# CMB-BNU/PloidyFrost

Measured on AMD Instinct MI355X. Metric: unitigs/s through superbubble+SeqAlign (k=25, z=8), higher is better.
Workload: dtype u64

## Files before the change

### ploidyfrost_amd/csrc/pf_call.hip

```cpp
#include "pf_call_kernels.hpp"
#include "pf_scan.hpp"

using namespace pf;

#define PF_TRY(call) do { const int s_ = (call); if (s_ != PF_OK) return s_; } while (0)

using namespace pf_call;

struct Need { DevBuf *buf; size_t bytes; };
static int need(pf_ctx *ctx, const char *who, std::initializer_list<Need> list) {
    for (const Need &n : list)
        if (!n.buf->ensure(n.bytes)) { pf::CtxErr{ctx} = std::string(who) + ": out of device memory"; return PF_ERR_HIP; }
    return PF_OK;
}

namespace pf {

void call_state_create(pf_ctx *ctx) { (void)state_of(ctx); }
void call_destroy(pf_ctx *ctx) {
    if (!ctx->call) return;
    ctx->call->release_all();
    delete ctx->call;
    ctx->call = nullptr;
}
// ... 242 lines not shown
    PF_HIP(hipMemcpyAsync(&total, S->side_base.as<uint32_t>() + N, 4, hipMemcpyDeviceToHost, st));
    PF_HIP(hipStreamSynchronize(st));
    S->n_sides = total;
    S->n_tasks = 0;
    S->low = lower;
    S->up = upper;
    *n_sides = total;
    if (total == 0) return PF_OK;
    if (!S->sides.ensure((size_t)total * sizeof(pf_call_side)) || !S->ctask.ensure((size_t)total * sizeof(CallTask)) ||
        !S->target.ensure((size_t)total * 4)) {
        pf::CtxErr{ctx} = "pf_call_scan: out of device memory";
        return PF_ERR_HIP;
    }
    ScanArgs a;
    a.flags = S->flags.as<uint8_t>(); a.plus = S->plus.as<uint32_t>(); a.minus = S->minus.as<uint32_t>();
    a.succ = ctx->d_succ; a.pred = ctx->d_pred; a.seq = ctx->d_seq; a.off = ctx->d_off; a.len = ctx->d_len; a.N = N; a.k = ctx->k;
    a.cov_sum = S->cov_sum.as<uint64_t>(); a.cov_min = S->cov_min.as<uint32_t>(); a.cov_miss = S->cov_miss.as<uint8_t>();
    a.per_strand = S->per_strand; a.low = lower; a.up = upper;
    a.side_base = S->side_base.as<uint32_t>(); a.sides = S->sides.as<pf_call_side>(); a.tasks = S->ctask.as<CallTask>();
    a.target = S->target.as<uint32_t>();
    a.n_colors = S->n_colors;
    a.ccov_sum = S->ccov_sum.as<uint64_t>(); a.ccov_min = S->ccov_min.as<uint32_t>(); a.ccov_max = S->ccov_max.as<uint32_t>(); a.ccov_miss = S->ccov_miss.as<uint8_t>();
    a.clow = S->col_low.as<uint32_t>(); a.cup = S->col_up.as<uint32_t>(); a.full = S->col_full.as<uint64_t>(); a.cwords = S->col_words; a.size_total = S->col_size.as<uint64_t>();
    ctx_begin(ctx, PF_K_CALL_SCAN);
    if (S->n_colors) k_call_sides<true><<<(N + 255) / 256, 256, 0, st>>>(a);
    else k_call_sides<false><<<(N + 255) / 256, 256, 0, st>>>(a);
    ctx_end(ctx);
    ctx_units(ctx, PF_K_CALL_SCAN, N);
    PF_HIP(hipGetLastError());
    return PF_OK;
}

int pf_call_resolve(pf_ctx *ctx, uint64_t *n_bubbles, uint32_t *err, uint32_t *err_unitig) {
    if (!ctx || !ctx->call || !n_bubbles || !err || !err_unitig) return PF_ERR_ARG;
    CallState *S = ctx->call;
    *n_bubbles = 0;
    *err = 0;
    *err_unitig = 0;
    S->n_tasks = 0;
    const uint64_t n = S->n_sides;
    if (n == 0) return PF_OK;
    PF_HIP(hipSetDevice(ctx->device));
    hipStream_t st = ctx->stream;
    if (!S->pending.ensure(n * 4) || !S->killed.ensure(n) || !S->rstate.ensure(n) || !S->rflag.ensure(n * 4) || !S->rsmall.ensure(64) ||
        !S->kept.ensure(n * 4)) {
        pf::CtxErr{ctx} = "pf_call_resolve: out of device memory";
// ... 878 lines not shown
```

### ploidyfrost_amd/csrc/pf_colored.hip

```cpp
#include <hip/hip_runtime.h>

#include <algorithm>
#include <cstdlib>
#include <cstring>
#include <string>
#include <vector>

#include "pf_colored_dev.hpp"
#include "pf_cov_stream.hpp"
#include "pf_ctx.hpp"
#include "pf_device_common.hpp"
#include "ploidyfrost_hip.h"

using namespace pf;

namespace {

constexpr uint32_t MISSING = pf::CTAB_MISSING;

__global__ void k_ctab_build(uint8_t *base, uint64_t mask, uint32_t line_bytes, int k, const uint64_t *__restrict__ kmers,
                             const uint32_t *__restrict__ counts, uint64_t n, uint64_t min_count, uint64_t max_count, uint32_t colour,
                             unsigned int *noncanon) {
    uint64_t i = (uint64_t)blockIdx.x * blockDim.x + threadIdx.x;
    const uint64_t stride = (uint64_t)gridDim.x * blockDim.x;
// ... 317 lines not shown
        ctx->n_colors, ctx->n_kmers, ctx->d_gcov_c, stride, rest, rest_n, rest_cap, ROWS)
        if (ctx->k == 25) PF_JOINC_LAUNCH(25);
        else if (ctx->k == 31) PF_JOINC_LAUNCH(31);
        else PF_JOINC_LAUNCH(0);
#undef PF_JOINC_LAUNCH
        ctx_end_at(ctx, at, st);
        (void)ctx_begin_at(ctx, PF_K_COV_JOIN_REST, st, &at);
        k_cov_join_colored_rest<<<blocks, 256, 0, st>>>(t, ctx->k, ctx->n_colors, rest, rest_n, rest_cap, ctx->d_gcov_c, stride, ctx->d_seq, ctx->d_off,
                                                                  ctx->d_kpre, ctx->d_khead, ctx->d_krow, ctx->n_kmers, ROWS);
        ctx_end_at(ctx, at, st);
    } else {
        (void)ctx_begin_at(ctx, PF_K_COV_JOIN, st, &at);
        k_cov_colored<<<ctx_grid(ctx, (uint64_t)ctx->N * 64, 256, 16), 256, 0, st>>>(t, ctx->d_seq, ctx->d_off, ctx->d_len, ctx->k, ctx->ctab_one_strand,
                                                                                            ctx->n_colors, 0, ctx->N, ctx->d_unread, nullptr, nullptr,
                                                                                            nullptr, nullptr, ctx->d_kpre, ctx->d_gcov_c, stride);
        ctx_end_at(ctx, at, st);
    }
    PF_HIP(hipGetLastError());
    PF_HIP(hipEventRecord(ctx->join_c_done, st));
    ctx->join_c_inflight = true;
    return PF_OK;
}

int join_colored_finish(pf_ctx *ctx) {
    if (!ctx->join_c_inflight) return PF_OK;
    ctx->join_c_inflight = false;
    PF_HIP(hipSetDevice(ctx->device));
    PF_HIP(hipEventSynchronize(ctx->join_c_done));
    ctx->gcov_c_valid = true;
    return PF_OK;
}

int join_graph_counts_colored(pf_ctx *ctx) {
    const int rc = join_graph_counts_colored_begin(ctx);
    return rc ? rc : join_colored_finish(ctx);
}
}

extern "C" {

uint32_t pf_num_colors(const pf_ctx *ctx) { return ctx ? ctx->n_colors : 0; }

int pf_upload_counts_colored(pf_ctx *ctx, uint32_t n_colors, const uint64_t *const *kmers, const uint32_t *const *counts,
                             const uint64_t *n, const uint64_t *min_count, const uint64_t *max_count, const int *both_strands) {
    if (!ctx || n_colors == 0 || !kmers || !counts || !n || !min_count || !max_count || !both_strands) return PF_ERR_ARG;
    if (n_colors > PF_MAX_COLORS_TABLE) { pf::CtxErr{ctx} = "more colours than the device table holds (PF_MAX_COLORS_TABLE)"; return PF_ERR_ARG; }
    if (!ctx->d_seq || !ctx->k) { pf::CtxErr{ctx} = "pf_upload_counts_colored: the graph comes first (the table is addressed by minimizers of length-k keys)"; return PF_ERR_ARG; }
    uint64_t total = 0, biggest = 0;
    for (uint32_t c = 0; c < n_colors; ++c) {
        if (n[c] && (!kmers[c] || !counts[c])) return PF_ERR_ARG;
        if (!both_strands[c]) continue;
        total += n[c];
        biggest = std::max(biggest, n[c]);
    }
    ctx->ctab_unread = 0;
    ctx->ctab_max_count = 0;
    std::vector<uint8_t> unread(n_colors, 0);
    for (uint32_t c = 0; c < n_colors; ++c) {
        if (!both_strands[c]) { unread[c] = 1; if (c < 64) ctx->ctab_unread |= 1ull << c; }
        else ctx->ctab_max_count = std::max<uint64_t>(ctx->ctab_max_count, max_count[c]);
    }
    (void)join_colored_finish(ctx);
    if (ctx->d_gcov_c) { (void)hipFree(ctx->d_gcov_c); ctx->d_gcov_c = nullptr; }
    ctx->gcov_c_valid = false;
    PF_HIP(hipSetDevice(ctx->device));
    if (ctx->d_ctab) { (void)hipFree(ctx->d_ctab); ctx->d_ctab = nullptr; }
    if (ctx->d_unread) { (void)hipFree(ctx->d_unread); ctx->d_unread = nullptr; }
    PF_HIP(hipMalloc(reinterpret_cast<void **>(&ctx->d_unread), n_colors));
    PF_HIP(hipMemcpy(ctx->d_unread, unread.data(), n_colors, hipMemcpyHostToDevice));
    ctx->n_colors = 0;
    uint64_t cap = 128;
    while (cap * 4 < biggest || cap * LINE_KEYS < total + total / 4 + 1) cap <<= 1;
    const uint32_t line_bytes = ctab_line_bytes(n_colors);
    PF_HIP(hipMalloc(reinterpret_cast<void **>(&ctx->d_ctab), cap * line_bytes));
    PF_HIP(hipMemsetAsync(ctx->d_ctab, 0xFF, cap * line_bytes, ctx->stream));
    ctx->ctab_cap = cap;
    ctx->ctab_line_bytes = line_bytes;
    DevTmp<unsigned int> noncanon_;
    PF_HIP(noncanon_.alloc(4));
    PF_HIP(hipMemsetAsync(noncanon_.p, 0, 4, ctx->stream));
    for (uint32_t c = 0; c < n_colors; ++c) {
        if (!n[c] || !both_strands[c]) continue;
        DevTmp<uint64_t> dk_;
        DevTmp<uint32_t> dc_;
        const uint64_t *pk = kmers[c];
// ... 28 lines not shown
    }
    ctx->n_colors = n_colors;
    return join_graph_counts_colored(ctx);
}

static int unitig_cov_colored_impl(pf_ctx *ctx, uint32_t u0, uint32_t u1, uint64_t *sum, uint32_t *mn, uint32_t *mx, uint8_t *miss, bool probe) {
    if (!ctx || !ctx->d_seq || !ctx->d_ctab || !ctx->n_colors || u0 > u1 || u1 > ctx->N || !sum || !mn || !mx || !miss) return PF_ERR_ARG;
    if (u0 == u1) return PF_OK;
    PF_HIP(hipSetDevice(ctx->device));
    const size_t n = (size_t)(u1 - u0) * ctx->n_colors;
    const bool dev_out = on_device(sum);
    uint64_t *ds = sum;
    uint32_t *dlo = mn, *dhi = mx;
    uint8_t *dx = miss;
    if (!dev_out) {
        ds = (uint64_t *)ctx_ws(ctx, WS_CCOV_SUM, n * 8);
        dlo = (uint32_t *)ctx_ws(ctx, WS_CCOV_MIN, n * 4);
        dhi = (uint32_t *)ctx_ws(ctx, WS_CCOV_MAX, n * 4);
        dx = (uint8_t *)ctx_ws(ctx, WS_CCOV_MISS, n);
        if (!ds || !dlo || !dhi || !dx) return PF_ERR_HIP;
    }
    constexpr bool env_probe = false;
    probe = probe || env_probe;
    { const int rc = join_colored_finish(ctx); if (rc) return rc; }
    if (!probe && !ctx->gcov_c_valid) {
        const int rc = join_graph_counts_colored(ctx);
        if (rc) return rc;
    }
    const bool stream = !probe && ctx->gcov_c_valid;
    uint64_t g_range[2] = {0, 0};
    if (stream) {
        PF_HIP(hipMemcpyAsync(&g_range[0], ctx->d_kpre + u0, 8, hipMemcpyDeviceToHost, ctx->stream));
        PF_HIP(hipMemcpyAsync(&g_range[1], ctx->d_kpre + u1, 8, hipMemcpyDeviceToHost, ctx->stream));
        PF_HIP(hipStreamSynchronize(ctx->stream));
    }
    ctx_begin(ctx, PF_K_COV_COLORED);
    if (stream) {
        k_ccov_init<<<ctx_grid(ctx, n, 256, 8), 256, 0, ctx->stream>>>(n, ds, dlo, dhi, dx);
        Kc4Args a{ctx->d_gcov_c, ctx->gcov_c_stride, ctx->d_unread, ctx->d_khead, ctx->d_krow, u0, u1 - u0, g_range[0], g_range[1],
                  g_range[0] / 256, (g_range[1] + 255) / 256, ds, dlo, dhi, dx};
        const int rc = launch_cov_stream(ctx, a, ctx->n_colors, ctx->ctab_max_count >= (1ull << 20), true);
        if (rc) return rc;
    } else {
        const CTab t{ctx->d_ctab, ctx->ctab_cap - 1, ctx->ctab_line_bytes};
        const int grid = ctx_grid(ctx, (uint64_t)(u1 - u0) * 64, 256, 16);
        k_cov_colored<<<grid, 256, 0, ctx->stream>>>(t, ctx->d_seq, ctx->d_off, ctx->d_len, ctx->k, ctx->ctab_one_strand, ctx->n_colors, u0, u1,
                                                     ctx->d_unread, ds, dlo, dhi, dx, nullptr, nullptr, 0);
    }
    ctx_end(ctx);
    if (!dev_out) {
        PF_HIP(hipMemcpyAsync(sum, ds, n * 8, hipMemcpyDeviceToHost, ctx->stream));
        PF_HIP(hipMemcpyAsync(mn, dlo, n * 4, hipMemcpyDeviceToHost, ctx->stream));
        PF_HIP(hipMemcpyAsync(mx, dhi, n * 4, hipMemcpyDeviceToHost, ctx->stream));
        PF_HIP(hipMemcpyAsync(miss, dx, n, hipMemcpyDeviceToHost, ctx->stream));
        PF_HIP(hipStreamSynchronize(ctx->stream));
    }
    return PF_OK;
}

int pf_unitig_cov_colored(pf_ctx *ctx, uint32_t u0, uint32_t u1, uint64_t *sum, uint32_t *mn, uint32_t *mx, uint8_t *miss) {
    return unitig_cov_colored_impl(ctx, u0, u1, sum, mn, mx, miss, false);
}

int pf_unitig_cov_colored_probe(pf_ctx *ctx, uint32_t u0, uint32_t u1, uint64_t *sum, uint32_t *mn, uint32_t *mx, uint8_t *miss) {
    return unitig_cov_colored_impl(ctx, u0, u1, sum, mn, mx, miss, true);
}

int pf_string_cov_colored(pf_ctx *ctx, const char *text, const uint64_t *str_off, uint32_t n_str, const uint32_t *low,
                          const uint32_t *up, uint64_t *sum, uint8_t *ok) {
    if (!ctx || !ctx->d_ctab || !ctx->n_colors || !low || !up || (n_str && (!text || !str_off || !sum || !ok))) return PF_ERR_ARG;
    if (n_str == 0) return PF_OK;
    PF_HIP(hipSetDevice(ctx->device));
    const uint32_t C = ctx->n_colors;
    uint64_t total = 0;
    PF_HIP(hipMemcpy(&total, str_off + n_str, 8, hipMemcpyDefault));
    char *dt = (char *)ctx_ws(ctx, WS_STR_TEXT, (size_t)total + 1);
    uint64_t *doff = (uint64_t *)ctx_ws(ctx, WS_STR_OFF, ((size_t)n_str + 1) * 8);
    uint64_t *ds = (uint64_t *)ctx_ws(ctx, WS_STR_SUM, (size_t)n_str * C * 8);
// ... 20 lines not shown
```

### ploidyfrost_amd/csrc/pf_ctx.hpp

```cpp
#pragma once
#include <hip/hip_runtime.h>
#include <stdint.h>

#include <mutex>
#include <string>
#include <vector>

#include "pf_device_common.hpp"
#include "ploidyfrost_hip.h"

namespace pf {
template <typename T>
struct DevTmp {
    T *p = nullptr;
    DevTmp() = default;
    DevTmp(const DevTmp &) = delete;
    DevTmp &operator=(const DevTmp &) = delete;
    ~DevTmp() { if (p) (void)hipFree(p); }
    hipError_t alloc(size_t bytes) { return hipMalloc(reinterpret_cast<void **>(&p), bytes ? bytes : 1); }
};

struct TimedLaunch {
    int kernel;
    hipEvent_t a, b;
// ... 19 lines not shown
    uint64_t *d_seq = nullptr;
    uint64_t *d_off = nullptr;
    uint32_t *d_len = nullptr;
    uint32_t N = 0;
    int k = 0;
    uint64_t n_words = 0, n_kmers = 0;
    uint64_t *d_kpre = nullptr;
    uint32_t *d_kwin = nullptr;
    uint64_t n_kwin = 0;
    uint32_t *d_succ = nullptr, *d_pred = nullptr;
    uint32_t *d_pred16 = nullptr;
    bool has_adj = false;
    uint32_t *d_cand = nullptr;
    std::vector<uint32_t> h_cand;
    std::vector<uint32_t> h_len;

    pf::CountLine *d_tab = nullptr;
    uint64_t tab_cap = 0, tab_n = 0;
    hipStream_t join_stream = nullptr;
    hipEvent_t join_done = nullptr;
    bool join_inflight = false;
    hipEvent_t join_c_done = nullptr;
    bool join_c_inflight = false;
    int tab_k = 0;
    bool tab_one_strand = false;
    bool tab_exact = false;
    uint64_t tab_max_count = 0;

    uint32_t *d_gcov = nullptr;
    uint64_t *d_khead = nullptr;
    uint32_t *d_krow = nullptr;
    uint64_t n_krow = 0;
    bool gcov_valid = false;

    uint8_t *d_ctab = nullptr;
    uint64_t ctab_cap = 0;
    uint32_t ctab_line_bytes = 128, n_colors = 0;
    bool ctab_one_strand = false;
    uint64_t ctab_unread = 0;
    uint8_t *d_unread = nullptr;
    uint64_t ctab_max_count = 0;
    uint32_t *d_gcov_c = nullptr;
    uint64_t gcov_c_stride = 0;
    bool gcov_c_valid = false;

    uint64_t *d_cov_sum = nullptr;
// ... 42 lines not shown
    size_t side_launch = (size_t)-1;
    size_t main_launch = (size_t)-1;
    std::mutex launch_mu;
    uint64_t units[PF_K_COUNT_] = {};
};

namespace pf {
struct CtxErr {
    pf_ctx *c;
    void operator=(std::string s) const {
        std::lock_guard<std::mutex> lk(c->launch_mu);
        c->err = std::move(s);
    }
};
#define PF_HIP(call)                                                                         \
    do {                                                                                     \
        hipError_t e_ = (call);                                                              \
        if (e_ != hipSuccess) {                                                              \
            pf::CtxErr{ctx} = std::string(#call) + ": " + hipGetErrorString(e_);                   \
            return PF_ERR_HIP;                                                               \
        }                                                                                    \
    } while (0)
struct Kc4Args;
int launch_cov_stream(pf_ctx *ctx, Kc4Args a, uint32_t n_colors, bool wide, bool colored);
int ctx_begin(pf_ctx *ctx, int kernel);
void ctx_end(pf_ctx *ctx);
int ctx_begin_on(pf_ctx *ctx, int kernel, hipStream_t stream);
void ctx_end_on(pf_ctx *ctx, hipStream_t stream);
int ctx_begin_at(pf_ctx *ctx, int kernel, hipStream_t stream, size_t *at);
void ctx_end_at(pf_ctx *ctx, size_t at, hipStream_t stream);
struct Timed {
    pf_ctx *ctx;
    Timed(pf_ctx *c, int kernel) : ctx(c) { ctx_begin(ctx, kernel); }
    ~Timed() { ctx_end(ctx); }
};
inline void ctx_units(pf_ctx *ctx, int kernel, uint64_t n) { if (ctx->timing) __atomic_fetch_add(&ctx->units[kernel], n, __ATOMIC_RELAXED); }
int ctx_grid(const pf_ctx *ctx, uint64_t work_items, int block, int per_cu);
inline size_t up256(size_t n) { return (n + 255) & ~(size_t)255; }
int join_graph_counts(pf_ctx *ctx);
int join_graph_counts_begin(pf_ctx *ctx);
int join_finish(pf_ctx *ctx);
int join_graph_counts_colored_begin(pf_ctx *ctx);
int join_colored_finish(pf_ctx *ctx);
hipStream_t join_stream(pf_ctx *ctx);
int join_graph_counts_colored(pf_ctx *ctx);
void *ctx_ws(pf_ctx *ctx, int slot, size_t bytes);
hipError_t lane_stream_create(hipStream_t *s, int lane);
struct DevLoadTrace {
    bool on = getenv("PF_TRACE_LOAD") != nullptr;
    std::chrono::steady_clock::time_point t = std::chrono::steady_clock::now();
    void mark(const char *what) {
        if (!on) return;
        const auto now = std::chrono::steady_clock::now();
        fprintf(stderr, "[load]   . %-42s %.3fs\n", what, std::chrono::duration<double>(now - t).count());
        t = now;
    }
};
void call_state_create(pf_ctx *ctx);
void call_destroy(pf_ctx *ctx);
void cc_destroy(pf_ctx *ctx);
void gfa_destroy(pf_ctx *ctx);
void comm_destroy(pf_ctx *ctx);
void count_destroy(pf_ctx *ctx);
void unitig_destroy(pf_ctx *ctx);
void clip_destroy(pf_ctx *ctx);
void call_invalidate(pf_ctx *ctx);
int call_state_arrays(pf_ctx *ctx, uint8_t **flags, uint32_t **plus, uint32_t **minus);
// ... 23 lines not shown
```

### ploidyfrost_amd/csrc/pf_device.hip

```cpp
#include <hip/hip_runtime.h>
#include <sys/mman.h>

#include <algorithm>
#include <cstdio>
#include <cstring>
#include <string>
#include <type_traits>
#include <vector>

#include "pf_cov_stream.hpp"
#include "pf_ctx.hpp"
#include "pf_device_common.hpp"
#include "pf_scan.hpp"
#include "ploidyfrost_hip.h"

using namespace pf;

static std::string g_create_err;


__global__ void k_fill_slots(Slot *t, uint64_t n) {
    uint64_t i = (uint64_t)blockIdx.x * blockDim.x + threadIdx.x;
    const uint64_t stride = (uint64_t)gridDim.x * blockDim.x;
    for (; i < n; i += stride) {
// ... 496 lines not shown
    w.first = p;
    w.second = want;
    return p;
}

hipError_t lane_stream_create(hipStream_t *s, int lane) {
    if (lane == 0) return hipStreamCreateWithFlags(s, hipStreamNonBlocking);
    int least = 0, greatest = 0;
    const hipError_t e = hipDeviceGetStreamPriorityRange(&least, &greatest);
    if (e != hipSuccess) return e;
    return hipStreamCreateWithPriority(s, hipStreamNonBlocking, least);
}

int ctx_grid(const pf_ctx *ctx, uint64_t work_items, int block, int per_cu) {
    uint64_t want = (work_items + block - 1) / block;
    uint64_t cap = (uint64_t)ctx->n_cu * per_cu;
    if (want < 1) want = 1;
    return (int)std::min<uint64_t>(want, cap);
}

}

namespace pf {
int launch_cov_stream(pf_ctx *ctx, Kc4Args a, uint32_t n_colors, bool wide, bool colored) {
    const uint64_t n_sr = a.sr_end - a.sr_begin;
    const dim3 grid((unsigned)(((n_sr + KC4_SR - 1) / KC4_SR + 3) / 4), n_colors);
    if (colored) {
        if (wide) k_cov_stream4<true, true><<<grid, 256, 0, ctx->stream>>>(a);
        else k_cov_stream4<false, true><<<grid, 256, 0, ctx->stream>>>(a);
    } else {
        if (wide) k_cov_stream4<true, false><<<grid, 256, 0, ctx->stream>>>(a);
        else k_cov_stream4<false, false><<<grid, 256, 0, ctx->stream>>>(a);
    }
    PF_HIP(hipGetLastError());
    return PF_OK;
}
}

namespace pf {
hipStream_t join_stream(pf_ctx *ctx) {
    if (!ctx->join_stream) {
        int least = 0, greatest = 0;
        (void)hipDeviceGetStreamPriorityRange(&least, &greatest);
        if (hipStreamCreateWithPriority(&ctx->join_stream, hipStreamNonBlocking, least) != hipSuccess) { (void)hipGetLastError(); ctx->join_stream = nullptr; }
    }
    return ctx->join_stream ? ctx->join_stream : ctx->stream;
}

int join_graph_counts_begin(pf_ctx *ctx) {
    ctx->gcov_valid = false;
    ctx->join_inflight = false;
    if (!ctx->d_seq || !ctx->d_tab || ctx->tab_exact || ctx->tab_max_count >= GCOV_MISSING || ctx->n_kmers == 0) return PF_OK;
    PF_HIP(hipSetDevice(ctx->device));
    if (!ctx->d_gcov && hipMalloc(&ctx->d_gcov, ((ctx->n_krow + 4) * 64) * sizeof(uint32_t)) != hipSuccess) {
        (void)hipGetLastError();
// ... 9 lines not shown
    uint32_t *rest_n = (uint32_t *)ctx_ws(ctx, WS_JOIN_REST_N, n_waves * 4);
    if (!rest || !rest_n) { pf::CtxErr{ctx} = "no room for K-COV-JOIN's hand-over list"; return PF_ERR_HIP; }
    if (!ctx->join_done) PF_HIP(hipEventCreateWithFlags(&ctx->join_done, hipEventDisableTiming));
    const hipStream_t st = join_stream(ctx);
    size_t at = 0;
    (void)ctx_begin_at(ctx, PF_K_COV_JOIN, st, &at);
#define PF_JOIN_LAUNCH(KK) k_cov_join<KK><<<blocks, 256, 0, st>>>(ctx->d_tab, ctx->tab_cap - 1, ctx->k, ctx->d_seq, ctx->d_off, ctx->d_kpre, ctx->d_khead, \
        ctx->d_krow, ctx->tab_one_strand, ctx->n_kmers, ctx->d_gcov, rest, rest_n, rest_cap, JOIN_ROWS_PER_WAVE)
    if (ctx->k == 25) PF_JOIN_LAUNCH(25);
    else if (ctx->k == 31) PF_JOIN_LAUNCH(31);
    else PF_JOIN_LAUNCH(0);
#undef PF_JOIN_LAUNCH
    ctx_end_at(ctx, at, st);
    (void)ctx_begin_at(ctx, PF_K_COV_JOIN_REST, st, &at);
    k_cov_join_rest<<<blocks, 256, 0, st>>>(ctx->d_tab, ctx->tab_cap - 1, ctx->k, ctx->tab_one_strand, rest, rest_n, rest_cap, ctx->d_gcov, ctx->d_seq, ctx->d_off,
                                            ctx->d_kpre, ctx->d_khead, ctx->d_krow, ctx->n_kmers, JOIN_ROWS_PER_WAVE);
    ctx_end_at(ctx, at, st);
    PF_HIP(hipGetLastError());
    PF_HIP(hipEventRecord(ctx->join_done, st));
    ctx->join_inflight = true;
    return PF_OK;
}

int join_finish(pf_ctx *ctx) {
    if (!ctx->join_inflight) return PF_OK;
    ctx->join_inflight = false;
    PF_HIP(hipSetDevice(ctx->device));
    PF_HIP(hipEventSynchronize(ctx->join_done));
    ctx->gcov_valid = true;
    return PF_OK;
}

int join_graph_counts(pf_ctx *ctx) {
    const int rc = join_graph_counts_begin(ctx);
    return rc ? rc : join_finish(ctx);
}
}

template <typename T>
static int stage_in(pf_ctx *ctx, const T *src, size_t n, T **dev, bool *owned) {
    *owned = false;
    if (n == 0) { *dev = nullptr; return PF_OK; }
    if (is_device_ptr(src)) {
        *dev = const_cast<T *>(src);
        return PF_OK;
    }
    PF_HIP(hipMalloc(dev, n * sizeof(T)));
    *owned = true;
    PF_HIP(hipMemcpyAsync(*dev, src, n * sizeof(T), hipMemcpyDefault, ctx->stream));
    return PF_OK;
}

extern "C" {

const char *pf_kernel_name(int kernel) { return (kernel >= 0 && kernel < PF_K_COUNT_) ? kKernelNames[kernel] : "?"; }

const char *pf_last_error(const pf_ctx *ctx) {
    if (!ctx) return g_create_err.c_str();
// ... 55 lines not shown
    hipFree(ctx->d_gcov); hipFree(ctx->d_khead); hipFree(ctx->d_krow); hipFree(ctx->d_gcov_c);
    ctx->d_gcov = nullptr;
    ctx->d_gcov_c = nullptr;
    ctx->gcov_c_valid = false;
    ctx->d_khead = nullptr;
    ctx->d_krow = nullptr;
    ctx->gcov_valid = false;
    ctx->d_kpre = nullptr;
    ctx->d_kwin = nullptr;
    ctx->d_pred16 = nullptr;
    ctx->d_seq = ctx->d_off = nullptr;
    ctx->d_len = ctx->d_succ = ctx->d_pred = ctx->d_cand = nullptr;
    ctx->h_cand.clear();
    ctx->has_adj = false;
}

void pf_destroy(pf_ctx *ctx) {
    if (!ctx) return;
    hipSetDevice(ctx->device);
    hipStreamSynchronize(ctx->stream);
    if (ctx->join_stream) { hipStreamSynchronize(ctx->join_stream); hipStreamDestroy(ctx->join_stream); }
    if (ctx->join_done) hipEventDestroy(ctx->join_done);
    if (ctx->join_c_done) hipEventDestroy(ctx->join_c_done);
    for (auto &tl : ctx->launches) { hipEventDestroy(tl.a); hipEventDestroy(tl.b); }
    for (auto &e : ctx->event_pool) hipEventDestroy(e);
    call_destroy(ctx);
    cc_destroy(ctx);
    gfa_destroy(ctx);
    comm_destroy(ctx);
    count_destroy(ctx);
    unitig_destroy(ctx);
    clip_destroy(ctx);
    free_graph(ctx);
    hipFree(ctx->d_tab);
    hipFree(ctx->d_ctab);
    hipFree(ctx->d_unread);
    hipFree(ctx->d_cov_sum); hipFree(ctx->d_cov_min); hipFree(ctx->d_cov_miss);
    for (auto &w : ctx->ws) hipFree(w.first);
    if (ctx->h_live) hipHostFree(ctx->h_live);
    if (ctx->copy_stream) { hipStreamSynchronize(ctx->copy_stream); hipStreamDestroy(ctx->copy_stream); }
    for (auto &lane : ctx->bub_streams) for (auto &s : lane) if (s) hipStreamDestroy(s);
    for (auto &lane : ctx->bub_events) for (auto &e : lane) if (e) hipEventDestroy(e);
    hipStreamDestroy(ctx->own_stream);
    delete ctx;
}

// ... 21 lines not shown
    return PF_OK;
}

int pf_reset_timing(pf_ctx *ctx) {
    if (!ctx) return PF_ERR_ARG;
    PF_HIP(hipSetDevice(ctx->device));
    PF_HIP(hipDeviceSynchronize());
    std::lock_guard<std::mutex> lk(ctx->launch_mu);
    for (auto &tl : ctx->launches) { ctx->event_pool.push_back(tl.a); ctx->event_pool.push_back(tl.b); }
    ctx->launches.clear();
    memset(ctx->units, 0, sizeof(ctx->units));
    return PF_OK;
}

int pf_kernel_units(pf_ctx *ctx, int kernel, uint64_t *units) {
    if (!ctx || kernel < 0 || kernel >= PF_K_COUNT_ || !units) return PF_ERR_ARG;
    *units = ctx->units[kernel];
    return PF_OK;
}

int pf_kernel_time(pf_ctx *ctx, int kernel, double *total_ms, uint64_t *launches) {
    if (!ctx || kernel < 0 || kernel >= PF_K_COUNT_) return PF_ERR_ARG;
    PF_HIP(hipStreamSynchronize(ctx->stream));
    double tot = 0;
    uint64_t n = 0;
    for (auto &tl : ctx->launches) {
        if (tl.kernel != kernel || !tl.closed) continue;
        float ms = 0;
        PF_HIP(hipEventElapsedTime(&ms, tl.a, tl.b));
        tot += ms;
        n++;
    }
    if (total_ms) *total_ms = tot;
    if (launches) *launches = n;
    return PF_OK;
}

static int busy_union(pf_ctx *ctx, uint64_t kernel_mask, double *busy_ms, double *span_ms) {
    if (!ctx) return PF_ERR_ARG;
    PF_HIP(hipSetDevice(ctx->device));
    PF_HIP(hipDeviceSynchronize());
    std::vector<std::pair<float, float>> iv;
    size_t unread = 0;
    {
        std::lock_guard<std::mutex> lk(ctx->launch_mu);
        iv.reserve(ctx->launches.size());
// ... 80 lines not shown

int pf_device_name(pf_ctx *ctx, char *buf, size_t cap) {
    if (!ctx || !buf || !cap) return PF_ERR_ARG;
    snprintf(buf, cap, "%s", ctx->name.c_str());
    return PF_OK;
}

int pf_device_pci_bus_id(pf_ctx *ctx, char *buf, size_t cap) {
    if (!ctx || !buf || cap < 16) return PF_ERR_ARG;
    PF_HIP(hipDeviceGetPCIBusId(buf, (int)cap, ctx->device));
    return PF_OK;
}

uint64_t pf_table_capacity(const pf_ctx *ctx) { return ctx ? ctx->tab_cap * pf::LINE_KEYS : 0; }
uint64_t pf_num_kmers(const pf_ctx *ctx) { return ctx ? ctx->n_kmers : 0; }

int pf_upload_graph(pf_ctx *ctx, const uint64_t *seq_words, const uint64_t *seq_off, const uint32_t *len_bp,
                    uint32_t N, int k) {
    if (!ctx || !seq_words || !seq_off || !len_bp || N == 0 || k < 3 || k > 31) return PF_ERR_ARG;
    if (N >= (1u << 30)) { pf::CtxErr{ctx} = "more than 2^30 unitigs"; return PF_ERR_ARG; }
    if (ctx->d_tab && ctx->tab_k != k) { pf::CtxErr{ctx} = "pf_upload_graph: k differs from the k of the resident count table"; return PF_ERR_ARG; }
    PF_HIP(hipSetDevice(ctx->device));
    DevLoadTrace trace;
    (void)join_finish(ctx);
    (void)join_colored_finish(ctx);
    free_graph(ctx);
    trace.mark("graph: previous graph released");
    uint64_t total_words = 0;
    PF_HIP(hipMemcpy(&total_words, seq_off + N, 8, hipMemcpyDefault));
    trace.mark("graph: size of the sequence array fetched");
    ctx->N = N;
    ctx->k = k;
    ctx->n_words = total_words;
    PF_HIP(hipMalloc(&ctx->d_seq, (total_words + 2) * 8));
    PF_HIP(hipMemsetAsync(ctx->d_seq, 0, (total_words + 2) * 8, ctx->stream));
    PF_HIP(hipMalloc(&ctx->d_off, ((size_t)N + 1) * 8));
    PF_HIP(hipMalloc(&ctx->d_len, (size_t)N * 4));
    trace.mark("graph: arrays allocated");
    PF_HIP(hipMemcpyAsync(ctx->d_seq, seq_words, total_words * 8, hipMemcpyDefault, ctx->stream));
    PF_HIP(hipMemcpyAsync(ctx->d_off, seq_off, ((size_t)N + 1) * 8, hipMemcpyDefault, ctx->stream));
    PF_HIP(hipMemcpyAsync(ctx->d_len, len_bp, (size_t)N * 4, hipMemcpyDefault, ctx->stream));
    PF_HIP(hipStreamSynchronize(ctx->stream));
    trace.mark("graph: arrays copied");
    {
        DevTmp<uint64_t> cnt_;
        DevTmp<unsigned int> bad_;
        PF_HIP(cnt_.alloc(((size_t)N + 1) * 8));
        PF_HIP(bad_.alloc(4));
// ... 162 lines not shown
    PF_HIP(hipStreamSynchronize(ctx->stream));
    return PF_OK;
}

static int check_table_strands(pf_ctx *ctx, bool keys_all_canonical) {
    ctx->tab_one_strand = false;
    if (!ctx->d_tab || !ctx->tab_n) return PF_OK;
    if (keys_all_canonical) { ctx->tab_one_strand = true; return PF_OK; }
    DevTmp<unsigned int> flag_;
    unsigned int h_flag = 0;
    PF_HIP(flag_.alloc(4));
    PF_HIP(hipMemsetAsync(flag_.p, 0, 4, ctx->stream));
    k_table_two_strands<<<ctx_grid(ctx, ctx->tab_cap * LINE_KEYS, 256, 8), 256, 0, ctx->stream>>>(ctx->d_tab, ctx->tab_cap, ctx->tab_k, flag_.p);
    PF_HIP(hipMemcpyAsync(&h_flag, flag_.p, 4, hipMemcpyDeviceToHost, ctx->stream));
    PF_HIP(hipStreamSynchronize(ctx->stream));
    ctx->tab_one_strand = h_flag == 0;
    return PF_OK;
}

int pf_upload_counts(pf_ctx *ctx, const uint64_t *kmers, const uint32_t *counts, uint64_t n, uint32_t k, uint64_t min_count,
                     uint64_t max_count, int both_strands) {
    if (!ctx || (n && (!kmers || !counts)) || k < 3 || k > 31) return PF_ERR_ARG;
    if (ctx->d_seq && (int)k != ctx->k) { pf::CtxErr{ctx} = "pf_upload_counts: k differs from the k of the resident graph"; return PF_ERR_ARG; }
    (void)join_finish(ctx);
    ctx->tab_exact = !both_strands;
    ctx->tab_max_count = max_count;
    call_invalidate(ctx);
    PF_HIP(hipSetDevice(ctx->device));
    hipFree(ctx->d_tab);
    ctx->d_tab = nullptr;
    hipFree(ctx->d_gcov);
    ctx->d_gcov = nullptr;
    ctx->gcov_valid = false;
    uint64_t cap = 128;
    while (cap * 4 < n) cap <<= 1;
    PF_HIP(hipMalloc(&ctx->d_tab, cap * sizeof(CountLine)));
    ctx->tab_cap = cap;
    ctx->tab_n = n;
    ctx->tab_k = (int)k;
    PF_HIP(hipMemsetAsync(ctx->d_tab, 0xFF, cap * sizeof(CountLine), ctx->stream));
    const bool on_dev = n && is_device_ptr(kmers);
    DevTmp<uint64_t> dk_;
    DevTmp<uint32_t> dc_;
    const uint64_t *pk = kmers;
    const uint32_t *pc = counts;
    if (!on_dev && n) {
        PF_HIP(dk_.alloc(n * 8));
// ... 2 lines not shown
        PF_HIP(hipMemcpyAsync(dc_.p, counts, n * 4, hipMemcpyDefault, ctx->stream));
        pk = dk_.p;
        pc = dc_.p;
    }
    DevTmp<unsigned int> noncanon_;
    unsigned int h_noncanon = 0;
    PF_HIP(noncanon_.alloc(4));
    PF_HIP(hipMemsetAsync(noncanon_.p, 0, 4, ctx->stream));
    if (n) {
        ctx_begin(ctx, PF_K_TABLE_BUILD);
        k_table_build<<<ctx_grid(ctx, n, 256, 8), 256, 0, ctx->stream>>>(ctx->d_tab, cap - 1, (int)k, pk, pc, n, min_count, max_count, noncanon_.p);
        ctx_end(ctx);
    }
    PF_HIP(hipMemcpyAsync(&h_noncanon, noncanon_.p, 4, hipMemcpyDeviceToHost, ctx->stream));
    PF_HIP(hipStreamSynchronize(ctx->stream));
    const int rc = check_table_strands(ctx, h_noncanon == 0);
    if (rc) return rc;
    if (ctx->d_seq && !ctx->tab_exact) return pf::join_graph_counts(ctx);
    return PF_OK;
}

int pf_release_counts(pf_ctx *ctx) {
    if (!ctx) return PF_ERR_ARG;
    (void)join_finish(ctx);
    call_invalidate(ctx);
    PF_HIP(hipSetDevice(ctx->device));
    hipFree(ctx->d_tab);
    ctx->d_tab = nullptr;
    hipFree(ctx->d_gcov);
    ctx->d_gcov = nullptr;
    ctx->gcov_valid = false;
    ctx->tab_cap = ctx->tab_n = 0;
    return PF_OK;
}

int pf_join_counts_begin(pf_ctx *ctx) {
    if (!ctx || !ctx->d_seq) return PF_ERR_ARG;
    const bool single = ctx->d_tab && !ctx->tab_exact, colored = ctx->d_ctab && ctx->n_colors;
    if (!single && !colored) { pf::CtxErr{ctx} = "pf_join_counts: no canonical count table resident"; return PF_ERR_ARG; }
    { const int rc = pf::join_finish(ctx); if (rc) return rc; }
    { const int rc = pf::join_colored_finish(ctx); if (rc) return rc; }
    if (single) {
        const int rc = pf::join_graph_counts_begin(ctx);
        if (rc) return rc;
        if (!ctx->join_inflight) { pf::CtxErr{ctx} = "pf_join_counts: no joined coverage array for this table (max_count = 2^32 - 1, or no room)"; return PF_ERR_ARG; }
    }
    if (colored) {
        const int rc = pf::join_graph_counts_colored_begin(ctx);
        if (rc) return rc;
        if (!ctx->join_c_inflight) { pf::CtxErr{ctx} = "pf_join_counts: no joined coverage array for these databases (max_count = 2^32 - 1, or no room)"; return PF_ERR_ARG; }
    }
    return PF_OK;
}

int pf_join_counts_end(pf_ctx *ctx) {
    if (!ctx) return PF_ERR_ARG;
    const int rc = pf::join_finish(ctx);
    return rc ? rc : pf::join_colored_finish(ctx);
}

int pf_join_counts(pf_ctx *ctx) {
    const int rc = pf_join_counts_begin(ctx);
    return rc ? rc : pf_join_counts_end(ctx);
}
// ... 21 lines not shown
    return PF_OK;
}

static int unitig_cov_impl(pf_ctx *ctx, uint32_t u0, uint32_t u1, int exact, uint64_t *sum, uint32_t *mn, uint8_t *miss, bool probe = false) {
    if (!ctx || !ctx->d_seq || !ctx->d_tab || u0 > u1 || u1 > ctx->N || !sum || !mn || !miss) return PF_ERR_ARG;
    if (u0 == u1) return PF_OK;
    PF_HIP(hipSetDevice(ctx->device));
    const uint32_t n = u1 - u0;
    const bool dev_out = is_device_ptr(sum);
    uint64_t *ds = sum;
    uint32_t *dm = mn;
    uint8_t *dx = miss;
    if (!dev_out) {
        if (ctx->cov_cap < n) {
            hipFree(ctx->d_cov_sum); hipFree(ctx->d_cov_min); hipFree(ctx->d_cov_miss);
            ctx->d_cov_sum = nullptr; ctx->d_cov_min = nullptr; ctx->d_cov_miss = nullptr;
            PF_HIP(hipMalloc(&ctx->d_cov_sum, (size_t)n * 8));
            PF_HIP(hipMalloc(&ctx->d_cov_min, (size_t)n * 4));
            PF_HIP(hipMalloc(&ctx->d_cov_miss, (size_t)n));
            ctx->cov_cap = n;
        }
        ds = ctx->d_cov_sum; dm = ctx->d_cov_min; dx = ctx->d_cov_miss;
    }
    uint64_t g_range[2];
    PF_HIP(hipMemcpyAsync(&g_range[0], ctx->d_kpre + u0, 8, hipMemcpyDeviceToHost, ctx->stream));
    PF_HIP(hipMemcpyAsync(&g_range[1], ctx->d_kpre + u1, 8, hipMemcpyDeviceToHost, ctx->stream));
    PF_HIP(hipStreamSynchronize(ctx->stream));
    const uint64_t w_begin = g_range[0] / KCOV_WIN, w_end = (g_range[1] + KCOV_WIN - 1) / KCOV_WIN;
    static const bool env_probe = [] { const char *e = getenv("PF_KCOV_SCAN"); return e && !strcmp(e, "probe"); }();
    probe = probe || env_probe;
    { const int rc = join_finish(ctx); if (rc) return rc; }
    if (!exact && !probe && !ctx->gcov_valid) {
        const int rc = join_graph_counts(ctx);
        if (rc) return rc;
    }
    ctx_begin(ctx, PF_K_COV);
    k_cov_init<<<ctx_grid(ctx, n, 256, 8), 256, 0, ctx->stream>>>(n, ds, dm, dx);
    if (!exact && !probe && ctx->gcov_valid) {
        Kc4Args a{ctx->d_gcov, 0, nullptr, ctx->d_khead, ctx->d_krow, u0, n, g_range[0], g_range[1], g_range[0] / 256, (g_range[1] + 255) / 256,
                  ds, dm, nullptr, dx};
        const bool wide = ctx->tab_max_count >= (1ull << 20);
        const int rc = launch_cov_stream(ctx, a, 1, wide, false);
        if (rc) return rc;
    } else {
        k_cov<<<ctx_grid(ctx, (w_end - w_begin) * 64, 256, 16), 256, 0, ctx->stream>>>(ctx->d_tab, ctx->tab_cap - 1, ctx->k, ctx->d_seq, ctx->d_off, ctx->d_kpre,
                                                                                     ctx->d_kwin, ctx->N, ctx->tab_one_strand, exact, u0, g_range[0],
                                                                                     g_range[1], w_begin, w_end - w_begin, ds, dm, dx, nullptr);
    }
    ctx_end(ctx);
    if (!dev_out) {
        PF_HIP(hipMemcpyAsync(sum, ds, (size_t)n * 8, hipMemcpyDeviceToHost, ctx->stream));
        PF_HIP(hipMemcpyAsync(mn, dm, (size_t)n * 4, hipMemcpyDeviceToHost, ctx->stream));
        PF_HIP(hipMemcpyAsync(miss, dx, (size_t)n, hipMemcpyDeviceToHost, ctx->stream));
        PF_HIP(hipStreamSynchronize(ctx->stream));
        for (uint32_t i = 0; i < n; ++i)
            if (miss[i]) { pf::CtxErr{ctx} = "a k-mer of the graph is missing from the count table"; return PF_ERR_MISSING_KMER; }
    }
    return PF_OK;
}

int pf_unitig_cov(pf_ctx *ctx, uint32_t u0, uint32_t u1, uint64_t *sum, uint32_t *mn, uint8_t *miss) {
    if (ctx && ctx->tab_exact) {
        pf::CtxErr{ctx} = "the count database was built without canonical counting: pf_unitig_cov_exact gives its per-orientation coverage";
        return PF_ERR_ARG;
    }
    return unitig_cov_impl(ctx, u0, u1, 0, sum, mn, miss);
}

int pf_unitig_cov_probe(pf_ctx *ctx, uint32_t u0, uint32_t u1, uint64_t *sum, uint32_t *mn, uint8_t *miss) {
    if (ctx && ctx->tab_exact) {
        pf::CtxErr{ctx} = "the count database was built without canonical counting: pf_unitig_cov_exact gives its per-orientation coverage";
        return PF_ERR_ARG;
    }
    return unitig_cov_impl(ctx, u0, u1, 0, sum, mn, miss, true);
}

int pf_unitig_cov_exact(pf_ctx *ctx, uint32_t u0, uint32_t u1, int reverse, uint64_t *sum, uint32_t *mn, uint8_t *miss) {
// ... 43 lines not shown
```

Baseline: 243.2 million.

## Run coverage kernels on the join stream with event gating instead of host syncs

```diff
diff --git a/ploidyfrost_amd/csrc/pf_call.hip b/ploidyfrost_amd/csrc/pf_call.hip
--- a/ploidyfrost_amd/csrc/pf_call.hip
+++ b/ploidyfrost_amd/csrc/pf_call.hip
@@ -288,6 +288,7 @@
     a.n_colors = S->n_colors;
     a.ccov_sum = S->ccov_sum.as<uint64_t>(); a.ccov_min = S->ccov_min.as<uint32_t>(); a.ccov_max = S->ccov_max.as<uint32_t>(); a.ccov_miss = S->ccov_miss.as<uint8_t>();
     a.clow = S->col_low.as<uint32_t>(); a.cup = S->col_up.as<uint32_t>(); a.full = S->col_full.as<uint64_t>(); a.cwords = S->col_words; a.size_total = S->col_size.as<uint64_t>();
+    if (ctx->cov_inflight) PF_HIP(hipStreamWaitEvent(st, ctx->cov_done, 0));
     ctx_begin(ctx, PF_K_CALL_SCAN);
     if (S->n_colors) k_call_sides<true><<<(N + 255) / 256, 256, 0, st>>>(a);
     else k_call_sides<false><<<(N + 255) / 256, 256, 0, st>>>(a);
diff --git a/ploidyfrost_amd/csrc/pf_colored.hip b/ploidyfrost_amd/csrc/pf_colored.hip
--- a/ploidyfrost_amd/csrc/pf_colored.hip
+++ b/ploidyfrost_amd/csrc/pf_colored.hip
@@ -363,6 +363,11 @@
     return PF_OK;
 }
 
+int join_colored_wait_on(pf_ctx *ctx, hipStream_t stream) {
+    if (ctx->join_c_inflight && stream != join_stream(ctx)) PF_HIP(hipStreamWaitEvent(stream, ctx->join_c_done, 0));
+    return PF_OK;
+}
+
 int join_colored_finish(pf_ctx *ctx) {
     if (!ctx->join_c_inflight) return PF_OK;
     ctx->join_c_inflight = false;
@@ -401,7 +406,7 @@
         if (!both_strands[c]) { unread[c] = 1; if (c < 64) ctx->ctab_unread |= 1ull << c; }
         else ctx->ctab_max_count = std::max<uint64_t>(ctx->ctab_max_count, max_count[c]);
     }
-    (void)join_colored_finish(ctx);
+    (void)join_drain(ctx);
     if (ctx->d_gcov_c) { (void)hipFree(ctx->d_gcov_c); ctx->d_gcov_c = nullptr; }
     ctx->gcov_c_valid = false;
     PF_HIP(hipSetDevice(ctx->device));
@@ -476,38 +481,43 @@
     }
     constexpr bool env_probe = false;
     probe = probe || env_probe;
-    { const int rc = join_colored_finish(ctx); if (rc) return rc; }
-    if (!probe && !ctx->gcov_c_valid) {
-        const int rc = join_graph_counts_colored(ctx);
+    if (!probe && !ctx->gcov_c_valid && !ctx->join_c_inflight) {
+        const int rc = join_graph_counts_colored_begin(ctx);
         if (rc) return rc;
     }
-    const bool stream = !probe && ctx->gcov_c_valid;
-    uint64_t g_range[2] = {0, 0};
-    if (stream) {
+    hipStream_t st;
+    { const int rc = cov_launch_begin(ctx, &st); if (rc) return rc; }
+    if (!probe) { const int rc = join_colored_wait_on(ctx, st); if (rc) return rc; }
+    const bool stream = !probe && (ctx->gcov_c_valid || ctx->join_c_inflight);
+    uint64_t g_range[2] = {0, ctx->n_kmers};
+    if (stream && (u0 != 0 || u1 != ctx->N)) {
         PF_HIP(hipMemcpyAsync(&g_range[0], ctx->d_kpre + u0, 8, hipMemcpyDeviceToHost, ctx->stream));
         PF_HIP(hipMemcpyAsync(&g_range[1], ctx->d_kpre + u1, 8, hipMemcpyDeviceToHost, ctx->stream));
         PF_HIP(hipStreamSynchronize(ctx->stream));
     }
-    ctx_begin(ctx, PF_K_COV_COLORED);
+    size_t at = 0;
+    (void)ctx_begin_at(ctx, PF_K_COV_COLORED, st, &at);
     if (stream) {
-        k_ccov_init<<<ctx_grid(ctx, n, 256, 8), 256, 0, ctx->stream>>>(n, ds, dlo, dhi, dx);
+        k_ccov_init<<<ctx_grid(ctx, n, 256, 8), 256, 0, st>>>(n, ds, dlo, dhi, dx);
         Kc4Args a{ctx->d_gcov_c, ctx->gcov_c_stride, ctx->d_unread, ctx->d_khead, ctx->d_krow, u0, u1 - u0, g_range[0], g_range[1],
                   g_range[0] / 256, (g_range[1] + 255) / 256, ds, dlo, dhi, dx};
-        const int rc = launch_cov_stream(ctx, a, ctx->n_colors, ctx->ctab_max_count >= (1ull << 20), true);
+        const int rc = launch_cov_stream(ctx, a, ctx->n_colors, ctx->ctab_max_count >= (1ull << 20), true, st);
         if (rc) return rc;
     } else {
         const CTab t{ctx->d_ctab, ctx->ctab_cap - 1, ctx->ctab_line_bytes};
         const int grid = ctx_grid(ctx, (uint64_t)(u1 - u0) * 64, 256, 16);
-        k_cov_colored<<<grid, 256, 0, ctx->stream>>>(t, ctx->d_seq, ctx->d_off, ctx->d_len, ctx->k, ctx->ctab_one_strand, ctx->n_colors, u0, u1,
-                                                     ctx->d_unread, ds, dlo, dhi, dx, nullptr, nullptr, 0);
-    }
-    ctx_end(ctx);
+        k_cov_colored<<<grid, 256, 0, st>>>(t, ctx->d_seq, ctx->d_off, ctx->d_len, ctx->k, ctx->ctab_one_strand, ctx->n_colors, u0, u1,
+                                            ctx->d_unread, ds, dlo, dhi, dx, nullptr, nullptr, 0);
+    }
+    ctx_end_at(ctx, at, st);
+    { const int rc = cov_launch_end(ctx, st); if (rc) return rc; }
     if (!dev_out) {
-        PF_HIP(hipMemcpyAsync(sum, ds, n * 8, hipMemcpyDeviceToHost, ctx->stream));
-        PF_HIP(hipMemcpyAsync(mn, dlo, n * 4, hipMemcpyDeviceToHost, ctx->stream));
-        PF_HIP(hipMemcpyAsync(mx, dhi, n * 4, hipMemcpyDeviceToHost, ctx->stream));
-        PF_HIP(hipMemcpyAsync(miss, dx, n, hipMemcpyDeviceToHost, ctx->stream));
-        PF_HIP(hipStreamSynchronize(ctx->stream));
+        PF_HIP(hipMemcpyAsync(sum, ds, n * 8, hipMemcpyDeviceToHost, st));
+        PF_HIP(hipMemcpyAsync(mn, dlo, n * 4, hipMemcpyDeviceToHost, st));
+        PF_HIP(hipMemcpyAsync(mx, dhi, n * 4, hipMemcpyDeviceToHost, st));
+        PF_HIP(hipMemcpyAsync(miss, dx, n, hipMemcpyDeviceToHost, st));
+        PF_HIP(hipStreamSynchronize(st));
+        ctx->cov_inflight = false;
     }
     return PF_OK;
 }
diff --git a/ploidyfrost_amd/csrc/pf_ctx.hpp b/ploidyfrost_amd/csrc/pf_ctx.hpp
--- a/ploidyfrost_amd/csrc/pf_ctx.hpp
+++ b/ploidyfrost_amd/csrc/pf_ctx.hpp
@@ -65,6 +65,9 @@
     bool join_inflight = false;
     hipEvent_t join_c_done = nullptr;
     bool join_c_inflight = false;
+    hipEvent_t cov_gate = nullptr;
+    hipEvent_t cov_done = nullptr;
+    bool cov_inflight = false;
     int tab_k = 0;
     bool tab_one_strand = false;
     bool tab_exact = false;
@@ -153,7 +156,7 @@
         }                                                                                    \
     } while (0)
 struct Kc4Args;
-int launch_cov_stream(pf_ctx *ctx, Kc4Args a, uint32_t n_colors, bool wide, bool colored);
+int launch_cov_stream(pf_ctx *ctx, Kc4Args a, uint32_t n_colors, bool wide, bool colored, hipStream_t stream);
 int ctx_begin(pf_ctx *ctx, int kernel);
 void ctx_end(pf_ctx *ctx);
 int ctx_begin_on(pf_ctx *ctx, int kernel, hipStream_t stream);
@@ -170,10 +173,15 @@
 inline size_t up256(size_t n) { return (n + 255) & ~(size_t)255; }
 int join_graph_counts(pf_ctx *ctx);
 int join_graph_counts_begin(pf_ctx *ctx);
+int join_graph_counts_colored_begin(pf_ctx *ctx);
+int join_wait_on(pf_ctx *ctx, hipStream_t stream);
+int join_colored_wait_on(pf_ctx *ctx, hipStream_t stream);
 int join_finish(pf_ctx *ctx);
-int join_graph_counts_colored_begin(pf_ctx *ctx);
 int join_colored_finish(pf_ctx *ctx);
+int join_drain(pf_ctx *ctx);
 hipStream_t join_stream(pf_ctx *ctx);
+int cov_launch_begin(pf_ctx *ctx, hipStream_t *stream);
+int cov_launch_end(pf_ctx *ctx, hipStream_t stream);
 int join_graph_counts_colored(pf_ctx *ctx);
 void *ctx_ws(pf_ctx *ctx, int slot, size_t bytes);
 hipError_t lane_stream_create(hipStream_t *s, int lane);
diff --git a/ploidyfrost_amd/csrc/pf_device.hip b/ploidyfrost_amd/csrc/pf_device.hip
--- a/ploidyfrost_amd/csrc/pf_device.hip
+++ b/ploidyfrost_amd/csrc/pf_device.hip
@@ -542,15 +542,15 @@
 }
 
 namespace pf {
-int launch_cov_stream(pf_ctx *ctx, Kc4Args a, uint32_t n_colors, bool wide, bool colored) {
+int launch_cov_stream(pf_ctx *ctx, Kc4Args a, uint32_t n_colors, bool wide, bool colored, hipStream_t stream) {
     const uint64_t n_sr = a.sr_end - a.sr_begin;
     const dim3 grid((unsigned)(((n_sr + KC4_SR - 1) / KC4_SR + 3) / 4), n_colors);
     if (colored) {
-        if (wide) k_cov_stream4<true, true><<<grid, 256, 0, ctx->stream>>>(a);
-        else k_cov_stream4<false, true><<<grid, 256, 0, ctx->stream>>>(a);
+        if (wide) k_cov_stream4<true, true><<<grid, 256, 0, stream>>>(a);
+        else k_cov_stream4<false, true><<<grid, 256, 0, stream>>>(a);
     } else {
-        if (wide) k_cov_stream4<true, false><<<grid, 256, 0, ctx->stream>>>(a);
-        else k_cov_stream4<false, false><<<grid, 256, 0, ctx->stream>>>(a);
+        if (wide) k_cov_stream4<true, false><<<grid, 256, 0, stream>>>(a);
+        else k_cov_stream4<false, false><<<grid, 256, 0, stream>>>(a);
     }
     PF_HIP(hipGetLastError());
     return PF_OK;
@@ -606,6 +606,11 @@
     return PF_OK;
 }
 
+int join_wait_on(pf_ctx *ctx, hipStream_t stream) {
+    if (ctx->join_inflight && stream != join_stream(ctx)) PF_HIP(hipStreamWaitEvent(stream, ctx->join_done, 0));
+    return PF_OK;
+}
+
 int join_finish(pf_ctx *ctx) {
     if (!ctx->join_inflight) return PF_OK;
     ctx->join_inflight = false;
@@ -618,6 +623,32 @@
 int join_graph_counts(pf_ctx *ctx) {
     const int rc = join_graph_counts_begin(ctx);
     return rc ? rc : join_finish(ctx);
+}
+
+int join_drain(pf_ctx *ctx) {
+    if (!ctx->join_stream && !ctx->join_inflight && !ctx->join_c_inflight && !ctx->cov_inflight) return PF_OK;
+    PF_HIP(hipSetDevice(ctx->device));
+    PF_HIP(hipStreamSynchronize(join_stream(ctx)));
+    ctx->cov_inflight = false;
+    const int rc = join_finish(ctx);
+    return rc ? rc : join_colored_finish(ctx);
+}
+
+int cov_launch_begin(pf_ctx *ctx, hipStream_t *stream) {
+    const hipStream_t st = *stream = join_stream(ctx);
+    if (st == ctx->stream) return PF_OK;
+    if (!ctx->cov_gate) PF_HIP(hipEventCreateWithFlags(&ctx->cov_gate, hipEventDisableTiming));
+    PF_HIP(hipEventRecord(ctx->cov_gate, ctx->stream));
+    PF_HIP(hipStreamWaitEvent(st, ctx->cov_gate, 0));
+    return PF_OK;
+}
+
+int cov_launch_end(pf_ctx *ctx, hipStream_t stream) {
+    PF_HIP(hipGetLastError());
+    if (!ctx->cov_done) PF_HIP(hipEventCreateWithFlags(&ctx->cov_done, hipEventDisableTiming));
+    PF_HIP(hipEventRecord(ctx->cov_done, stream));
+    ctx->cov_inflight = true;
+    return PF_OK;
 }
 }
 
@@ -719,6 +750,8 @@
     if (ctx->join_stream) { hipStreamSynchronize(ctx->join_stream); hipStreamDestroy(ctx->join_stream); }
     if (ctx->join_done) hipEventDestroy(ctx->join_done);
     if (ctx->join_c_done) hipEventDestroy(ctx->join_c_done);
+    if (ctx->cov_gate) hipEventDestroy(ctx->cov_gate);
+    if (ctx->cov_done) hipEventDestroy(ctx->cov_done);
     for (auto &tl : ctx->launches) { hipEventDestroy(tl.a); hipEventDestroy(tl.b); }
     for (auto &e : ctx->event_pool) hipEventDestroy(e);
     call_destroy(ctx);
@@ -786,6 +819,7 @@
 int pf_kernel_time(pf_ctx *ctx, int kernel, double *total_ms, uint64_t *launches) {
     if (!ctx || kernel < 0 || kernel >= PF_K_COUNT_) return PF_ERR_ARG;
     PF_HIP(hipStreamSynchronize(ctx->stream));
+    if (ctx->join_stream) PF_HIP(hipStreamSynchronize(ctx->join_stream));
     double tot = 0;
     uint64_t n = 0;
     for (auto &tl : ctx->launches) {
@@ -912,8 +946,7 @@
     if (ctx->d_tab && ctx->tab_k != k) { pf::CtxErr{ctx} = "pf_upload_graph: k differs from the k of the resident count table"; return PF_ERR_ARG; }
     PF_HIP(hipSetDevice(ctx->device));
     DevLoadTrace trace;
-    (void)join_finish(ctx);
-    (void)join_colored_finish(ctx);
+    (void)join_drain(ctx);
     free_graph(ctx);
     trace.mark("graph: previous graph released");
     uint64_t total_words = 0;
@@ -1122,7 +1155,7 @@
                      uint64_t max_count, int both_strands) {
     if (!ctx || (n && (!kmers || !counts)) || k < 3 || k > 31) return PF_ERR_ARG;
     if (ctx->d_seq && (int)k != ctx->k) { pf::CtxErr{ctx} = "pf_upload_counts: k differs from the k of the resident graph"; return PF_ERR_ARG; }
-    (void)join_finish(ctx);
+    (void)join_drain(ctx);
     ctx->tab_exact = !both_strands;
     ctx->tab_max_count = max_count;
     call_invalidate(ctx);
@@ -1171,7 +1204,7 @@
 
 int pf_release_counts(pf_ctx *ctx) {
     if (!ctx) return PF_ERR_ARG;
-    (void)join_finish(ctx);
+    (void)join_drain(ctx);
     call_invalidate(ctx);
     PF_HIP(hipSetDevice(ctx->device));
     hipFree(ctx->d_tab);
@@ -1187,8 +1220,6 @@
     if (!ctx || !ctx->d_seq) return PF_ERR_ARG;
     const bool single = ctx->d_tab && !ctx->tab_exact, colored = ctx->d_ctab && ctx->n_colors;
     if (!single && !colored) { pf::CtxErr{ctx} = "pf_join_counts: no canonical count table resident"; return PF_ERR_ARG; }
-    { const int rc = pf::join_finish(ctx); if (rc) return rc; }
-    { const int rc = pf::join_colored_finish(ctx); if (rc) return rc; }
     if (single) {
         const int rc = pf::join_graph_counts_begin(ctx);
         if (rc) return rc;
@@ -1256,37 +1287,46 @@
         }
         ds = ctx->d_cov_sum; dm = ctx->d_cov_min; dx = ctx->d_cov_miss;
     }
-    uint64_t g_range[2];
-    PF_HIP(hipMemcpyAsync(&g_range[0], ctx->d_kpre + u0, 8, hipMemcpyDeviceToHost, ctx->stream));
-    PF_HIP(hipMemcpyAsync(&g_range[1], ctx->d_kpre + u1, 8, hipMemcpyDeviceToHost, ctx->stream));
-    PF_HIP(hipStreamSynchronize(ctx->stream));
+    uint64_t g_range[2] = {0, ctx->n_kmers};
+    if (u0 != 0 || u1 != ctx->N) {
+        PF_HIP(hipMemcpyAsync(&g_range[0], ctx->d_kpre + u0, 8, hipMemcpyDeviceToHost, ctx->stream));
+        PF_HIP(hipMemcpyAsync(&g_range[1], ctx->d_kpre + u1, 8, hipMemcpyDeviceToHost, ctx->stream));
+        PF_HIP(hipStreamSynchronize(ctx->stream));
+    }
     const uint64_t w_begin = g_range[0] / KCOV_WIN, w_end = (g_range[1] + KCOV_WIN - 1) / KCOV_WIN;
     static const bool env_probe = [] { const char *e = getenv("PF_KCOV_SCAN"); return e && !strcmp(e, "probe"); }();
     probe = probe || env_probe;
-    { const int rc = join_finish(ctx); if (rc) return rc; }
-    if (!exact && !probe && !ctx->gcov_valid) {
-        const int rc = join_graph_counts(ctx);
+    const bool joined = !exact && !probe;
+    if (joined && !ctx->gcov_valid && !ctx->join_inflight) {
+        const int rc = join_graph_counts_begin(ctx);
         if (rc) return rc;
     }
-    ctx_begin(ctx, PF_K_COV);
-    k_cov_init<<<ctx_grid(ctx, n, 256, 8), 256, 0, ctx->stream>>>(n, ds, dm, dx);
-    if (!exact && !probe && ctx->gcov_valid) {
+    hipStream_t st;
+    { const int rc = cov_launch_begin(ctx, &st); if (rc) return rc; }
+    if (joined) { const int rc = join_wait_on(ctx, st); if (rc) return rc; }
+    const bool streamed = joined && (ctx->gcov_valid || ctx->join_inflight);
+    size_t at = 0;
+    (void)ctx_begin_at(ctx, PF_K_COV, st, &at);
+    k_cov_init<<<ctx_grid(ctx, n, 256, 8), 256, 0, st>>>(n, ds, dm, dx);
+    if (streamed) {
         Kc4Args a{ctx->d_gcov, 0, nullptr, ctx->d_khead, ctx->d_krow, u0, n, g_range[0], g_range[1], g_range[0] / 256, (g_range[1] + 255) / 256,
                   ds, dm, nullptr, dx};
         const bool wide = ctx->tab_max_count >= (1ull << 20);
-        const int rc = launch_cov_stream(ctx, a, 1, wide, false);
+        const int rc = launch_cov_stream(ctx, a, 1, wide, false, st);
         if (rc) return rc;
     } else {
-        k_cov<<<ctx_grid(ctx, (w_end - w_begin) * 64, 256, 16), 256, 0, ctx->stream>>>(ctx->d_tab, ctx->tab_cap - 1, ctx->k, ctx->d_seq, ctx->d_off, ctx->d_kpre,
-                                                                                     ctx->d_kwin, ctx->N, ctx->tab_one_strand, exact, u0, g_range[0],
-                                                                                     g_range[1], w_begin, w_end - w_begin, ds, dm, dx, nullptr);
-    }
-    ctx_end(ctx);
+        k_cov<<<ctx_grid(ctx, (w_end - w_begin) * 64, 256, 16), 256, 0, st>>>(ctx->d_tab, ctx->tab_cap - 1, ctx->k, ctx->d_seq, ctx->d_off, ctx->d_kpre,
+                                                                             ctx->d_kwin, ctx->N, ctx->tab_one_strand, exact, u0, g_range[0],
+                                                                             g_range[1], w_begin, w_end - w_begin, ds, dm, dx, nullptr);
+    }
+    ctx_end_at(ctx, at, st);
+    { const int rc = cov_launch_end(ctx, st); if (rc) return rc; }
     if (!dev_out) {
-        PF_HIP(hipMemcpyAsync(sum, ds, (size_t)n * 8, hipMemcpyDeviceToHost, ctx->stream));
-        PF_HIP(hipMemcpyAsync(mn, dm, (size_t)n * 4, hipMemcpyDeviceToHost, ctx->stream));
-        PF_HIP(hipMemcpyAsync(miss, dx, (size_t)n, hipMemcpyDeviceToHost, ctx->stream));
-        PF_HIP(hipStreamSynchronize(ctx->stream));
+        PF_HIP(hipMemcpyAsync(sum, ds, (size_t)n * 8, hipMemcpyDeviceToHost, st));
+        PF_HIP(hipMemcpyAsync(mn, dm, (size_t)n * 4, hipMemcpyDeviceToHost, st));
+        PF_HIP(hipMemcpyAsync(miss, dx, (size_t)n, hipMemcpyDeviceToHost, st));
+        PF_HIP(hipStreamSynchronize(st));
+        ctx->cov_inflight = false;
         for (uint32_t i = 0; i < n; ++i)
             if (miss[i]) { pf::CtxErr{ctx} = "a k-mer of the graph is missing from the count table"; return PF_ERR_MISSING_KMER; }
     }
```

Result: no change. 241.5 million (-0.7%).
